# baggepinnen/LPVSpectral.jl

Measured on AMD Instinct MI355X. Metric: signals/sec, ls_sparse_spectral_lpv group lasso N=2^20 Nf=512 Nv=8 (2000 ADMM iters; iters/sec in admm_iters_per_sec), higher is better.
Workload: dtype f64

## Files before the change

### lpvspectral.jl_amd/csrc/api.hip

```cpp
#include <cmath>
#include <cstdarg>
#include <cstdio>
#include <cstdlib>
#include <cstring>
#include <ctime>
#include <map>
#include <mutex>
#include <array>
#include <thread>
#include <string>
#include <vector>

#include "lpvs_internal.h"

namespace lpvs {

static thread_local char g_err[512] = "";

void set_error(const char *fmt, ...) {
    va_list ap;
    va_start(ap, fmt);
    vsnprintf(g_err, sizeof(g_err), fmt, ap);
    va_end(ap);
}
// ... 872 lines not shown
    sl.s0 = sl.nf8;
    bool merged = false;
    if (Nf > 1 && D != 0.0L) {
        const long double j0r = 2.0L * a0 / D;
        const long long j0 = llroundl(j0r);
        const long double delta = 2.0L * a0 - (long double)j0 * D;
        if (j0 >= 0 && j0 < Nf && std::fabs((double)delta) * xam <= 1e-7) {
            merged = true; sl.merged = true;
            sl.s0 = j0; sl.delta = (double)delta;
            sl.nsl = round_up(j0 + 2 * Nf - 1, 8);
            sl.s8 = sl.nsl;
        }
    }
    sl.om_hi.resize((size_t)sl.nsl); sl.om_lo.resize((size_t)sl.nsl);
    if (merged) {
        for (int64_t j = 0; j < sl.nsl; ++j) split((long double)j * D, sl.om_hi[j], sl.om_lo[j]);
    } else {
        for (int64_t m = 0; m < sl.nf8; ++m) split((long double)m * D, sl.om_hi[m], sl.om_lo[m]);
        for (int64_t q = 0; q < sl.s8; ++q) split(2.0L * a0 + (long double)q * D, sl.om_hi[sl.nf8 + q], sl.om_lo[sl.nf8 + q]);
    }
    for (int64_t f = 0; f < sl.nf8; ++f) split(a0 + (long double)f * D, sl.omr_hi[f], sl.omr_lo[f]);
    for (int b = 0; b < 8; ++b) split((long double)b * D, sl.step.hi[b], sl.step.lo[b]);
    return sl;
}
struct ApSlotsDev {
    DevBuf hi, lo, rhi, rlo, eps;
    int32_t upload(const ApSlots &sl, hipStream_t s) {
        LPVS_TRY(hi.alloc(sizeof(double) * (size_t)sl.nsl)); LPVS_TRY(lo.alloc(sizeof(double) * (size_t)sl.nsl));
        LPVS_TRY(rhi.alloc(sizeof(double) * (size_t)sl.nf8)); LPVS_TRY(rlo.alloc(sizeof(double) * (size_t)sl.nf8));
        LPVS_TRY(eps.alloc(sizeof(double) * sl.eps.size()));
        LPVS_TRY(copy_to_device(hi.p, sl.om_hi.data(), sizeof(double) * (size_t)sl.nsl, s));
        LPVS_TRY(copy_to_device(lo.p, sl.om_lo.data(), sizeof(double) * (size_t)sl.nsl, s));
        LPVS_TRY(copy_to_device(rhi.p, sl.omr_hi.data(), sizeof(double) * (size_t)sl.nf8, s));
        LPVS_TRY(copy_to_device(rlo.p, sl.omr_lo.data(), sizeof(double) * (size_t)sl.nf8, s));
        LPVS_TRY(copy_to_device(eps.p, sl.eps.data(), sizeof(double) * sl.eps.size(), s));
        return LPVS_OK;
    }
};

static int32_t create_lpv_impl(const double *y, int64_t ns, const double *X, const double *V, int64_t N, const double *w, int64_t Nf,
                               int64_t Nv, int32_t normalize, int32_t coulomb, int32_t device, lpvs_problem **out,
                               const double *ranges = nullptr) {
    if (N <= 0 || Nf <= 0 || Nv <= 0 || ns <= 0) { set_error("N, Nf, Nv and the number of signals must be positive"); return LPVS_EARGUMENT; }
    lpvs_problem *h = nullptr;
    LPVS_TRY(problem_begin(device, out, &h));
    struct Guard { lpvs_problem *h; ~Guard() { delete h; } } guard{h};
    hipStream_t s = h->stream;
    const int64_t nb = coulomb ? 2 * Nv : Nv;
    h->kind = 1; h->N = N; h->Nf = Nf; h->nb = nb; h->n = 2 * Nf * nb; h->np = round_up(h->n, 128); h->ns = ns;
    DevArg dy, dX, dV, dw;
    LPVS_TRY(dy.set(y, N * ns, s)); LPVS_TRY(dX.set(X, N, s)); LPVS_TRY(dV.set(V, N, s)); LPVS_TRY(dw.set(w, Nf, s));
    LPVS_TRY(h->G.alloc(sizeof(double) * (size_t)h->np * (size_t)h->np));
    LPVS_TRY(h->b.alloc(sizeof(double) * (size_t)h->np * (size_t)ns));
    LPVS_HIP(hipMemsetAsync(h->G.p, 0, h->G.bytes, s));
    LPVS_HIP(hipMemsetAsync(h->b.p, 0, h->b.bytes, s));
    LPVS_TRY(alloc_state(h));

    const int form_opt = option_in_effect(LPVS_OPT_GRAM_FORM, h->opt[LPVS_OPT_GRAM_FORM]);
    const std::string form = form_opt == LPVS_GRAM_AP ? "ap" : form_opt == LPVS_GRAM_KRS ? "krs" : form_opt == LPVS_GRAM_KR ? "kr" : "auto";
    bool use_ap = false;
    ApSlots sl;
    double xam = 0;
    if (form == "auto" || form == "ap") {
        std::vector<double> hw;
        LPVS_TRY(fetch_host(hw, w, Nf));
        double xlo, xhi;
        if (ranges) xam = ranges[3];
        else LPVS_TRY(device_minmax(dX.p, N, &xlo, &xhi, &xam, s));
        sl = make_ap_slots(hw, xam);
        use_ap = sl.ok;
        if (form == "ap" && !use_ap) { set_error("LPVS_GRAM_FORM=ap but w is not an arithmetic progression (max|eps|*max|x| = %.3g)", sl.emax * xam); return LPVS_EARGUMENT; }
    }
    if (use_ap) {
        const int64_t nf8 = sl.nf8, nsl = sl.nsl, P = nb * (nb + 1) / 2;
        const ApStep &step = sl.step;
        double lo, hi, am, gamma; std::vector<double> vc;
        DevBuf K, KK, dvc, part, tab, tabb, nwork, epsr;
        ApSlotsDev sd;
        DrainOnExit drain(s);
        LPVS_HIP(hipEventRecord(h->ev[0].a, s));
        if (ranges) { lo = ranges[0]; hi = ranges[1]; am = ranges[2]; }
        else LPVS_TRY(device_minmax(dV.p, N, &lo, &hi, &am, s));
        basis_centers(lo, hi, am, Nv, coulomb, vc, &gamma);
        const int64_t ldk = nb + 1;
        LPVS_TRY(dvc.alloc(sizeof(double) * vc.size()));
        LPVS_TRY(copy_to_device(dvc.p, vc.data(), sizeof(double) * vc.size(), s));
        LPVS_TRY(K.alloc(sizeof(double) * (size_t)N * (size_t)ldk));
        LPVS_TRY(KK.alloc(sizeof(double) * (size_t)N * (size_t)P));
        LPVS_TRY(launch_basis_table(dV.p, N, dvc.as<double>(), nb, gamma, normalize, coulomb, K.as<double>(), ldk, s));
        LPVS_TRY(launch_pair_table(K.as<double>(), ldk, nb, N, KK.as<double>(), s));
        LPVS_TRY(sd.upload(sl, s));
        LPVS_HIP(hipEventRecord(h->ev[0].b, s));
        LPVS_TRY(part.alloc(std::max(nudft_partial_bytes(N, nsl, P), nudft_partial_bytes(N, nf8, nb))));
        LPVS_TRY(tab.alloc(sizeof(double) * (size_t)nsl * (size_t)P * 4));
        LPVS_TRY(tabb.alloc(sizeof(double) * (size_t)nf8 * (size_t)nb * 4));
        LPVS_HIP(hipEventRecord(h->ev[1].a, s));
        const bool nufft_on = option_in_effect(LPVS_OPT_SLOT_SUMS, h->opt[LPVS_OPT_SLOT_SUMS]) != LPVS_SLOTS_DIRECT;
        bool nufft = nufft_on && sl.merged && nufft_applicable(N, nsl, P);
        const int nfg = nufft_grid_size(nsl);
        const double xam_ = xam;
        if (nufft) {
            LPVS_TRY(nwork.alloc(nufft_work_bytes(N, nsl, P)));
            const int32_t rc = launch_nufft_tab(dX.p, nullptr, N, xam_, KK.as<double>(), P, (int)P, step.hi[1], step.lo[1], 0, (int)nsl, nfg, false, nwork.p,
                                                tab.as<double>(), s);
            if (rc == kNufftNonFinite) nufft = false;
            else if (rc != LPVS_OK) return rc;
        }
        if (nufft) {
            h->gram_form = 5;
        } else {
            h->gram_form = 4;
            LPVS_TRY(launch_nudft(dX.p, nullptr, N, KK.as<double>(), P, (int)P, sd.hi.as<double>(), sd.lo.as<double>(), (int)nsl, step, part.as<double>(), tab.as<double>(), s));
        }
        LPVS_TRY(launch_ap_assemble(tab.as<double>(), sd.eps.as<double>(), Nf, sl.s0, sl.delta, nb, h->n, h->G.as<double>(), h->np, s));
        LPVS_HIP(hipEventRecord(h->ev[1].b, s));
        LPVS_HIP(hipEventRecord(h->ev[2].a, s));
        const bool nufft_rhs = nufft && sl.s0 % 2 == 0 && (int)(sl.s0 / 2 + nf8) <= (int)nsl;
        if (nufft_rhs) {
            std::vector<double> er(sl.eps.size());
            for (size_t f = 0; f < er.size(); ++f) er[f] = sl.eps[f] + 0.5 * sl.delta;
            LPVS_TRY(epsr.alloc(sizeof(double) * er.size()));
            LPVS_TRY(copy_to_device(epsr.p, er.data(), sizeof(double) * er.size(), s));
            LPVS_HIP(hipStreamSynchronize(s));
        }
// ... 1527 lines not shown
```

### lpvspectral.jl_amd/csrc/nudft.hip

```cpp
#include "lpvs_internal.h"

#include <cstdlib>

namespace lpvs {

namespace {

constexpr int RB = 16;

template <int QPT, int S>
__global__ void __launch_bounds__(256)
nudft_accumulate_kernel(const double *__restrict__ x, const double *__restrict__ y, int64_t N, const double *__restrict__ Wt,
                        int64_t ldw, int nq, const double *__restrict__ om_hi, const double *__restrict__ om_lo, int nslots,
                        const ApStep step, double *__restrict__ out, const int64_t *__restrict__ seg, int64_t rows_per_chunk) {
    constexpr int SLOTS = 64 * S, NA = 8 * S;
    constexpr int WSTR = (QPT + 1) & ~1;
    constexpr int NEF = NA + 8;
    __shared__ __attribute__((aligned(16))) double wrow[2][RB][4 * WSTR];
    __shared__ __attribute__((aligned(16))) double ef[2][RB][NEF][2];
    __shared__ double xs[2][RB], ys[2][RB];
    const int t = threadIdx.x;
    const int sl = t & 63;
    const int g = __builtin_amdgcn_readfirstlane(t >> 6);
    const int slot0 = blockIdx.x * SLOTS;
// ... 181 lines not shown
    }
}

__global__ void __launch_bounds__(256)
nudft_reduce_kernel(const double *__restrict__ part_all, int nchunks, int64_t count, double *__restrict__ out_all) {
    const int64_t i = (int64_t)blockIdx.x * 256 + threadIdx.x;
    if (i >= count) return;
    const double *part = part_all + (int64_t)blockIdx.y * nchunks * count;
    double s = 0;
    for (int c = 0; c < nchunks; ++c) s += part[(int64_t)c * count + i];
    out_all[(int64_t)blockIdx.y * count + i] = s;
}

__global__ void __launch_bounds__(256)
ap_assemble_fourier_kernel(const double *__restrict__ tab_all, const double *__restrict__ eps, int Nf, int s0, double delta, int zf, double scale,
                           int64_t n, double *__restrict__ G_all, int64_t ldg, int64_t tab_stride, int64_t g_stride) {
    const int64_t ga = blockIdx.y;
    const int64_t gb = (int64_t)blockIdx.x * 256 + threadIdx.x;
    if (gb > ga || ga >= n) return;
    const double *tab = tab_all + (int64_t)blockIdx.z * tab_stride;
    double *G = G_all + (int64_t)blockIdx.z * g_stride;
    const int ca = ga >= Nf, cb = gb >= Nf;
    const int ka = ca ? (int)ga - Nf + zf : (int)ga, kb = cb ? (int)gb - Nf + zf : (int)gb;
    const int hi = ka >= kb ? ka : kb, lo = ka >= kb ? kb : ka;
    const double dm = eps[hi] - eps[lo], dp = (eps[ka] + eps[kb]) + delta;
    const double *tm = tab + (int64_t)(hi - lo) * 4;
    const double *tp = tab + (int64_t)(s0 + ka + kb) * 4;
    const double cm = fma(-dm, tm[3], tm[0]);
    double sm = fma(dm, tm[2], tm[1]);
    if (ka < kb) sm = -sm;
    const double cp = fma(-dp, tp[3], tp[0]), sp = fma(dp, tp[2], tp[1]);
    double v;
    if (!ca && !cb) v = 0.5 * (cm + cp);
    else if (ca && cb) v = 0.5 * (cm - cp);
    else if (!ca && cb) v = -0.5 * (sp - sm);
    else v = -0.5 * (sp + sm);
    v *= scale;
    G[ga * ldg + gb] = v;
    G[gb * ldg + ga] = v;
}

__global__ void __launch_bounds__(256)
ap_rhs_fourier_kernel(const double *__restrict__ tab_all, const double *__restrict__ eps, int Nf, int zf, double dd,
                      double *__restrict__ b_all, int64_t tab_stride, int64_t b_stride) {
    const int k = blockIdx.x * 256 + threadIdx.x;
    if (k >= Nf) return;
    const double *t = tab_all + (int64_t)blockIdx.y * tab_stride + (int64_t)k * 4;
    double *b = b_all + (int64_t)blockIdx.y * b_stride;
    const double e = eps[k];
    b[k] = dd * fma(-e, t[3], t[0]);
    if (k >= zf) b[Nf + k - zf] = -dd * fma(e, t[2], t[1]);
}

__global__ void __launch_bounds__(256)
ap_assemble_kernel(const double *__restrict__ tab, const double *__restrict__ eps, int Nf, int s0, double delta, int nb, int P, int64_t n,
                   double *__restrict__ G, int64_t ldg) {
    const int64_t ga = blockIdx.y;
    const int64_t gb = (int64_t)blockIdx.x * 256 + threadIdx.x;
    if (gb > ga || ga >= n) return;
    const int g2 = 2 * nb;
    const int fa = (int)(ga / g2), ra = (int)(ga - (int64_t)fa * g2), ca = ra >= nb, ja0 = ra - ca * nb;
    const int fb = (int)(gb / g2), rbm = (int)(gb - (int64_t)fb * g2), cb = rbm >= nb, jb0 = rbm - cb * nb;
    int ja = ja0, jb = jb0;
    if (ja > jb) { const int t = ja; ja = jb; jb = t; }
    const int q = ja * nb - ja * (ja - 1) / 2 + (jb - ja);
    const int m = fa - fb, s = fa + fb;
    const double dm = eps[fa] - eps[fb], dp = (eps[fa] + eps[fb]) + delta;
    const double *tm = tab + ((int64_t)m * P + q) * 4;
    const double *tp = tab + ((int64_t)(s0 + s) * P + q) * 4;
    const double cm = fma(-dm, tm[3], tm[0]), sm = fma(dm, tm[2], tm[1]);
    const double cp = fma(-dp, tp[3], tp[0]), sp = fma(dp, tp[2], tp[1]);
    double v;
    if (!ca && !cb) v = 0.5 * (cm + cp);
    else if (ca && cb) v = 0.5 * (cm - cp);
    else if (!ca && cb) v = -0.5 * (sp - sm);
    else v = -0.5 * (sp + sm);
    G[ga * ldg + gb] = v;
    G[gb * ldg + ga] = v;
}

__global__ void __launch_bounds__(256)
ap_rhs_kernel(const double *__restrict__ tab, const double *__restrict__ eps, int Nf, int nb, double *__restrict__ b) {
    const int i = blockIdx.x * 256 + threadIdx.x;
    if (i >= Nf * nb) return;
    const int f = i / nb, j = i - f * nb;
    const double *t = tab + ((int64_t)f * nb + j) * 4;
    const double e = eps[f];
    b[(int64_t)f * 2 * nb + j] = fma(-e, t[3], t[0]);
    b[(int64_t)f * 2 * nb + nb + j] = -fma(e, t[2], t[1]);
}

template <int QPT, int S>
void launch_accumulate(unsigned nchunks, hipStream_t s, const double *x, const double *y, int64_t N, const double *Wt, int64_t ldw, int nq,
                       const double *om_hi, const double *om_lo, int nslots, const ApStep &step, double *partial, const int64_t *seg,
                       int64_t rpc) {
    dim3 grid((unsigned)ceil_div(nslots, 64 * S), nchunks, (unsigned)ceil_div(nq, 4 * QPT));
    hipLaunchKernelGGL((nudft_accumulate_kernel<QPT, S>), grid, dim3(256), 0, s, x, y, N, Wt, ldw, nq, om_hi, om_lo, nslots, step, partial, seg, rpc);
}

}

int64_t nudft_rows_per_chunk(int64_t N, int64_t nslots) {
    const int64_t groups = ceil_div(nslots, 128);
    int64_t rpc = 8192;
    while (rpc > 64 && groups * ceil_div(N, rpc) < 2048) rpc >>= 1;
    return rpc;
}
size_t nudft_chunks(int64_t N, int64_t nslots) { return (size_t)ceil_div(N, nudft_rows_per_chunk(N, nslots)); }
size_t nudft_partial_bytes(int64_t N, int64_t nslots, int64_t nq) {
    return sizeof(double) * nudft_chunks(N, nslots) * (size_t)nslots * (size_t)nq * 4;
}

static int32_t nudft_impl(const double *x, const double *y, int64_t N, const double *Wt, int64_t ldw, int nq, const double *om_hi,
                          const double *om_lo, int nslots, const ApStep &step, double *partial, double *tab, const int64_t *seg,
                          unsigned nseg, unsigned nbatch, hipStream_t s) {
    if (nslots % 8 != 0) { set_error("nudft: slot count %d is not a multiple of 8", nslots); return LPVS_ESTATE; }
    const unsigned nchunks = seg ? nseg : (unsigned)nudft_chunks(N, nslots);
    const int64_t rpc = seg ? 0 : nudft_rows_per_chunk(N, nslots);
    if (nq == 1) {
        dim3 grid((unsigned)ceil_div(nslots, 128), nchunks, 1);
        hipLaunchKernelGGL(nudft_single_kernel<2>, grid, dim3(256), 0, s, x, y, N, Wt, ldw, om_hi, om_lo, nslots, step, partial, seg, rpc);
    } else if (nq <= 8) launch_accumulate<2, 2>(nchunks, s, x, y, N, Wt, ldw, nq, om_hi, om_lo, nslots, step, partial, seg, rpc);
    else if (nq <= 16) launch_accumulate<4, 2>(nchunks, s, x, y, N, Wt, ldw, nq, om_hi, om_lo, nslots, step, partial, seg, rpc);
    else launch_accumulate<9, 2>(nchunks, s, x, y, N, Wt, ldw, nq, om_hi, om_lo, nslots, step, partial, seg, rpc);
    LPVS_HIP(hipGetLastError());
    const int64_t count = (int64_t)nslots * nq * 4;
    hipLaunchKernelGGL(nudft_reduce_kernel, dim3((unsigned)ceil_div(count, 256), nbatch), dim3(256), 0, s, partial, (int)(nchunks / nbatch), count, tab);
    LPVS_HIP(hipGetLastError());
    return LPVS_OK;
}

int32_t launch_nudft(const double *x, const double *y, int64_t N, const double *Wt, int64_t ldw, int nq, const double *om_hi,
                     const double *om_lo, int nslots, const ApStep &step, double *partial, double *tab, hipStream_t s) {
    return nudft_impl(x, y, N, Wt, ldw, nq, om_hi, om_lo, nslots, step, partial, tab, nullptr, 0, 1, s);
}

int32_t launch_nudft_windows(const double *x, const double *y, const double *Wt, const double *om_hi, const double *om_lo, int nslots,
                             const ApStep &step, const int64_t *seg_dev, int nwin, int segs_per_window, double *partial, double *tab,
                             hipStream_t s) {
    return nudft_impl(x, y, 0, Wt, 1, 1, om_hi, om_lo, nslots, step, partial, tab, seg_dev, (unsigned)(nwin * segs_per_window), (unsigned)nwin, s);
}

int32_t launch_ap_assemble_fourier(const double *tab, const double *eps, int64_t Nf, int64_t s0, double delta, int zf, int64_t n, double *G,
                                   int64_t ldg, int nbatch, int64_t tab_stride, int64_t g_stride, hipStream_t s) {
    dim3 grid((unsigned)ceil_div(n, 256), (unsigned)n, (unsigned)nbatch);
    hipLaunchKernelGGL(ap_assemble_fourier_kernel, grid, dim3(256), 0, s, tab, eps, (int)Nf, (int)s0, delta, zf, 1.0 / (double)(2 * Nf), n, G, ldg,
                       tab_stride, g_stride);
    LPVS_HIP(hipGetLastError());
    return LPVS_OK;
}

int32_t launch_ap_rhs_fourier(const double *tab, const double *eps, int64_t Nf, int zf, double *b, int nbatch, int64_t tab_stride,
                              int64_t b_stride, hipStream_t s) {
    hipLaunchKernelGGL(ap_rhs_fourier_kernel, dim3((unsigned)ceil_div(Nf, 256), (unsigned)nbatch), dim3(256), 0, s, tab, eps, (int)Nf, zf,
                       1.0 / sqrt((double)(2 * Nf)), b, tab_stride, b_stride);
    LPVS_HIP(hipGetLastError());
    return LPVS_OK;
}

int32_t launch_ap_assemble(const double *tab, const double *eps, int64_t Nf, int64_t s0, double delta, int64_t nb, int64_t n, double *G,
                           int64_t ldg, hipStream_t s) {
    const int P = (int)(nb * (nb + 1) / 2);
    dim3 grid((unsigned)ceil_div(n, 256), (unsigned)n);
    hipLaunchKernelGGL(ap_assemble_kernel, grid, dim3(256), 0, s, tab, eps, (int)Nf, (int)s0, delta, (int)nb, P, n, G, ldg);
    LPVS_HIP(hipGetLastError());
    return LPVS_OK;
}

int32_t launch_ap_rhs(const double *tab, const double *eps, int64_t Nf, int64_t nb, double *b, hipStream_t s) {
    hipLaunchKernelGGL(ap_rhs_kernel, dim3((unsigned)ceil_div(Nf * nb, 256)), dim3(256), 0, s, tab, eps, (int)Nf, (int)nb, b);
    LPVS_HIP(hipGetLastError());
    return LPVS_OK;
}

}
```

### lpvspectral.jl_amd/csrc/nufft.hip

```cpp
#include "lpvs_internal.h"

#include <cmath>
#include <map>
#include <mutex>
#include <vector>

namespace lpvs {
namespace {

constexpr int NU_W = 16;
constexpr double NU_BETA = 2.30 * NU_W;
static int nu_gpw(int nf) { return nf <= 4096 ? 4 : 2; }
constexpr double NU_MAGIC = 6755399441055744.0;
constexpr int NU_CHUNK = 32768;

__global__ void __launch_bounds__(256)
nufft_coord_kernel(const double *__restrict__ x, int64_t N, double D_hi, double D_lo, int nf, int *__restrict__ cell0, double *__restrict__ taps) {
    const int64_t i = (int64_t)blockIdx.x * 256 + threadIdx.x;
    if (i >= N) return;
    constexpr double I2PI_HI = 0.15915494309189535, I2PI_LO = -9.8393384885635288e-18;
    const double xv = x[i];
    const double th = D_hi * xv, tl = fma(D_hi, xv, -th) + D_lo * xv;
    const double uh = th * I2PI_HI, ul = fma(th, I2PI_HI, -uh) + (th * I2PI_LO + tl * I2PI_HI);
    double r = (uh - rint(uh)) + ul;
    r -= floor(r);
    double p = r * (double)nf;
    if (p >= (double)nf) p -= (double)nf;
    const int g0 = (int)ceil(p - 0.5 * NU_W);
    cell0[i] = (g0 + nf) & (nf - 1);
#pragma unroll
    for (int k = 0; k < NU_W; ++k) {
        const double z = ((double)(g0 + k) - p) * (2.0 / NU_W);
        const double s = 1.0 - z * z;
        taps[i * NU_W + k] = s > 0.0 ? exp(NU_BETA * (sqrt(s) - 1.0)) : exp(-NU_BETA);
    }
}

__global__ void __launch_bounds__(256)
nufft_colmax_kernel(const double *__restrict__ Wt, const double *__restrict__ y, int64_t ldw, int nq, int64_t N, unsigned long long *__restrict__ out) {
    __shared__ unsigned long long m[256];
    for (int q = threadIdx.x; q < 256; q += 256) m[q] = 0;
    __syncthreads();
    const int64_t total = N * ldw;
    for (int64_t e = (int64_t)blockIdx.x * 256 + threadIdx.x; e < total; e += (int64_t)gridDim.x * 256) {
        const int q = (int)(e % ldw);
        if (q < nq) {
            const double v = fabs(y ? Wt[e] * y[e / ldw] : Wt[e]);
            if (v > 0.0 || v != v) atomicMax(&m[q & 255], v != v ? 0x7ff0000000000000ull : (unsigned long long)__double_as_longlong(v));
        }
    }
    __syncthreads();
    for (int q = threadIdx.x; q < nq && q < 256; q += 256) if (m[q]) atomicMax(out + q, m[q]);
}

template <int GPW>
__global__ void __launch_bounds__(256)
nufft_spread_kernel(const double *__restrict__ x, const double *__restrict__ y, const double *__restrict__ Wt, int64_t ldw, int nq, int64_t N, int nf,
                    const int *__restrict__ cell0, const double *__restrict__ taps, const double *__restrict__ invq,
                    long long *__restrict__ partial, int ngroups, int nchunks) {
    extern __shared__ __attribute__((aligned(16))) long long G[];
    const int xcd = blockIdx.x & 7, jj = blockIdx.x >> 3;
    const int gg = jj % ngroups, ch = xcd + 8 * (jj / ngroups);
    if (ch >= nchunks) return;
    for (int e = threadIdx.x; e < GPW * nf; e += 256) G[e] = 0;
    __syncthreads();
    constexpr int NC = GPW / 2;
    const int q0 = gg * NC;
    double iq[GPW];
#pragma unroll
    for (int c = 0; c < NC; ++c) { iq[2 * c] = q0 + c < nq ? invq[2 * (q0 + c)] : 0.0; iq[2 * c + 1] = q0 + c < nq ? invq[2 * (q0 + c) + 1] : 0.0; }
    const int64_t n0 = (int64_t)ch * NU_CHUNK, n1 = n0 + NU_CHUNK < N ? n0 + NU_CHUNK : N;
    const long long magic_bits = __double_as_longlong(NU_MAGIC);
    for (int64_t n = n0 + threadIdx.x; n < n1; n += 256) {
        const int c0 = cell0[n];
        const double xv = x[n], yv = y ? y[n] : 1.0;
        double cw[GPW];
#pragma unroll
        for (int c = 0; c < NC; ++c) {
            const double wv = q0 + c < nq ? Wt[n * ldw + q0 + c] * yv : 0.0;
            cw[2 * c] = wv * iq[2 * c];
            cw[2 * c + 1] = (xv * wv) * iq[2 * c + 1];
        }
        const double2 *tp = reinterpret_cast<const double2 *>(taps + n * NU_W);
#pragma unroll
        for (int k2 = 0; k2 < NU_W / 2; ++k2) {
            const double2 t = tp[k2];
#pragma unroll
            for (int h = 0; h < 2; ++h) {
                const double tv = h ? t.y : t.x;
                const int cell = (c0 + 2 * k2 + h) & (nf - 1);
#pragma unroll
                for (int gi = 0; gi < GPW; ++gi) {
                    const long long a = __double_as_longlong(fma(cw[gi], tv, NU_MAGIC)) - magic_bits;
                    atomicAdd(reinterpret_cast<unsigned long long *>(&G[gi * nf + cell]), (unsigned long long)a);
                }
            }
        }
    }
    __syncthreads();
    long long *out = partial + ((int64_t)ch * ngroups + gg) * GPW * nf;
    for (int e = threadIdx.x; e < GPW * nf; e += 256) out[e] = G[e];
}

__global__ void __launch_bounds__(256)
nufft_reduce_kernel(const long long *__restrict__ partial, int ngroups, int nchunks, int nf, int gpw, double *__restrict__ grid) {
    const int gamma = blockIdx.y, q = gamma >> 1, twin = gamma & 1;
    const int gg = q / (gpw / 2), gi = (q % (gpw / 2)) * 2 + twin;
    const int g = blockIdx.x * 256 + threadIdx.x;
    if (g >= nf) return;
    long long s = 0;
    for (int ch = 0; ch < nchunks; ++ch) s += partial[(((int64_t)ch * ngroups + gg) * gpw + gi) * nf + g];
    grid[(int64_t)gamma * nf + g] = (double)s;
}

template <bool HALF>
__global__ void __launch_bounds__(256)
nufft_modes_kernel(const double *__restrict__ grid, int nf, int nq, int mode0, int nslots,
                   const double *__restrict__ scale , double *__restrict__ tab,
                   int64_t scale_stride , int64_t grid_bstride, int64_t tab_bstride ) {
    grid += (int64_t)blockIdx.z * grid_bstride;
    tab += (int64_t)blockIdx.z * tab_bstride;
    extern __shared__ __attribute__((aligned(16))) double lds[];
    double *Gd = lds;
    double2 *tw = reinterpret_cast<double2 *>(lds + nf);
    const int gamma = blockIdx.x, q = gamma >> 1, twin = gamma & 1;
    const int ntw = HALF ? nf >> 1 : nf;
    for (int g = threadIdx.x; g < nf; g += 256) {
        Gd[g] = grid[(int64_t)gamma * nf + g];
        if (g < ntw) {
            double sn, cs;
            sincospi(2.0 * (double)g / (double)nf, &sn, &cs);
            tw[g] = make_double2(cs, sn);
        }
    }
    __syncthreads();
    const int j = blockIdx.y * 256 + threadIdx.x;
    if (j >= nslots) return;
    double ac0 = 0, as0 = 0, ac1 = 0, as1 = 0;
    int idx = 0;
    const int mask = nf - 1, mj = (mode0 + j) & mask;
    const int hmask = mask >> 1, hbit = nf >> 1;
    for (int g = 0; g < nf; g += 2) {
        const double2 t0 = tw[HALF ? idx & hmask : idx];
        const bool n0 = HALF && (idx & hbit);
        idx = (idx + mj) & mask;
        const double2 t1 = tw[HALF ? idx & hmask : idx];
        const bool n1 = HALF && (idx & hbit);
        idx = (idx + mj) & mask;
        double v0 = Gd[g], v1 = Gd[g + 1];
        if (HALF) { v0 = n0 ? -v0 : v0; v1 = n1 ? -v1 : v1; }
        ac0 = fma(v0, t0.x, ac0); as0 = fma(v0, t0.y, as0);
        ac1 = fma(v1, t1.x, ac1); as1 = fma(v1, t1.y, as1);
    }
    const double sc = scale[(int64_t)gamma * scale_stride + j];
// ... 75 lines not shown
    }
}

}

static std::vector<long double> nufft_phihat(int nf, int nmodes) {
    static const std::vector<std::pair<long double, long double>> gl = [] {
        const int n = 96;
        std::vector<std::pair<long double, long double>> r((size_t)n);
        const long double pi = 3.141592653589793238462643383279502884L;
        for (int i = 0; i < n; ++i) {
            long double z = cosl(pi * (i + 0.75L) / (n + 0.5L)), pp = 0;
            for (int it = 0; it < 100; ++it) {
                long double p1 = 1, p2 = 0;
                for (int k = 1; k <= n; ++k) { const long double p3 = p2; p2 = p1; p1 = ((2 * k - 1) * z * p2 - (k - 1) * p3) / k; }
                pp = n * (z * p1 - p2) / (z * z - 1);
                const long double dz = p1 / pp;
                z -= dz;
                if (fabsl(dz) < 1e-19L) break;
            }
            r[(size_t)i] = {z, 2 / ((1 - z * z) * pp * pp)};
        }
        return r;
    }();
    static std::mutex phat_mu;
    static std::map<std::pair<int, int>, std::vector<long double>> phat_cache;
    std::lock_guard<std::mutex> lk(phat_mu);
    auto it = phat_cache.find({nf, nmodes});
    if (it == phat_cache.end()) {
        std::vector<long double> v((size_t)nmodes);
        const long double pi = 3.141592653589793238462643383279502884L, half = 0.5L * NU_W;
        for (int j = 0; j < nmodes; ++j) {
            long double acc = 0;
            for (const auto &nw : gl) {
                const long double z = nw.first, t = z * half;
                acc += nw.second * half * expl((long double)NU_BETA * (sqrtl(1 - z * z) - 1)) * cosl(2 * pi * (long double)j * t / (long double)nf);
            }
            v[(size_t)j] = acc;
        }
        it = phat_cache.emplace(std::make_pair(nf, nmodes), std::move(v)).first;
    }
    return it->second;
}

int nufft_grid_size(int64_t nslots) {
    int nf = 256;
    while ((double)nf < 3.9 * (double)nslots) nf *= 2;
    return nf;
}
bool nufft_applicable(int64_t N, int64_t nslots, int64_t nq) {
    const int nf = nufft_grid_size(nslots);
    return nf <= 8192 && N >= 4096 && nq >= 1 && nq <= 256;
}
size_t nufft_work_bytes(int64_t N, int64_t nslots, int64_t nq) {
    const int nf = nufft_grid_size(nslots), gpw = nu_gpw(nf);
    const int64_t ngroups = (nq + gpw / 2 - 1) / (gpw / 2), nchunks = (N + NU_CHUNK - 1) / NU_CHUNK;
    size_t b = 0;
    b += sizeof(double) * (size_t)N * NU_W;
    b += ((sizeof(int) * (size_t)N + 255) / 256) * 256;
    b += sizeof(long long) * (size_t)nchunks * (size_t)ngroups * (size_t)gpw * (size_t)nf;
    b += sizeof(double) * (size_t)(2 * nq) * (size_t)(nslots + 1);
    b += sizeof(double) * (size_t)(2 * nq) * (size_t)nf;
    b += sizeof(unsigned long long) * (size_t)nq + 256;
    return b;
}

int32_t launch_nufft_tab(const double *x, const double *y, int64_t N, double xam, const double *Wt, int64_t ldw, int nq, double D_hi, double D_lo,
                         int mode0, int nslots, int nf, bool reuse_coords, void *work, double *tab, hipStream_t s) {
    const int gpw = nu_gpw(nf);
    const int ngroups = (nq + gpw / 2 - 1) / (gpw / 2), nchunks = (int)((N + NU_CHUNK - 1) / NU_CHUNK);
    unsigned char *wp = static_cast<unsigned char *>(work);
    double *taps = reinterpret_cast<double *>(wp); wp += sizeof(double) * (size_t)N * NU_W;
    int *cell0 = reinterpret_cast<int *>(wp); wp += ((sizeof(int) * (size_t)N + 255) / 256) * 256;
    long long *partial = reinterpret_cast<long long *>(wp); wp += sizeof(long long) * (size_t)nchunks * (size_t)ngroups * (size_t)gpw * (size_t)nf;
    double *scale = reinterpret_cast<double *>(wp); wp += sizeof(double) * (size_t)(2 * nq) * (size_t)nslots;
    double *invq = reinterpret_cast<double *>(wp); wp += sizeof(double) * (size_t)(2 * nq);
    double *grid = reinterpret_cast<double *>(wp); wp += sizeof(double) * (size_t)(2 * nq) * (size_t)nf;
    unsigned long long *colmax = reinterpret_cast<unsigned long long *>(wp);

    LPVS_HIP(hipMemsetAsync(colmax, 0, sizeof(unsigned long long) * (size_t)nq, s));
    if (!reuse_coords) hipLaunchKernelGGL(nufft_coord_kernel, dim3((unsigned)ceil_div(N, 256)), dim3(256), 0, s, x, N, D_hi, D_lo, nf, cell0, taps);
    if (nq > 256) { set_error("nufft: more than 256 weight vectors"); return LPVS_EUNSUPPORTED; }
    hipLaunchKernelGGL(nufft_colmax_kernel, dim3(1024), dim3(256), 0, s, Wt, y, ldw, nq, N, colmax);
    LPVS_HIP(hipGetLastError());
    std::vector<unsigned long long> hm((size_t)nq);
    LPVS_HIP(hipMemcpyAsync(hm.data(), colmax, sizeof(unsigned long long) * (size_t)nq, hipMemcpyDeviceToHost, s));
    LPVS_HIP(hipStreamSynchronize(s));
    for (int q = 0; q < nq; ++q)
        if (!std::isfinite(__builtin_bit_cast(double, hm[(size_t)q])) || !std::isfinite(xam)) return kNufftNonFinite;
    std::vector<double> hscale((size_t)(2 * nq) * (size_t)nslots), hinvq((size_t)(2 * nq));
    const std::vector<long double> phat = nufft_phihat(nf, mode0 + nslots);
    for (int q = 0; q < nq; ++q) {
        const double cmax = __builtin_bit_cast(double, hm[(size_t)q]);
        for (int twin = 0; twin < 2; ++twin) {
            const double bound = (twin ? xam : 1.0) * cmax * (double)N;
            int e = 0;
            (void)std::frexp(bound > 0 ? bound : 1.0, &e);
            const double quantum = std::ldexp(1.0, e - 62);
            hinvq[(size_t)(2 * q + twin)] = bound > 0 ? 1.0 / quantum : 0.0;
            for (int j = 0; j < nslots; ++j) hscale[(size_t)(2 * q + twin) * (size_t)nslots + (size_t)j] = (double)((long double)quantum / phat[(size_t)(mode0 + j)]);
        }
    }
    LPVS_TRY(copy_to_device(scale, hscale.data(), sizeof(double) * hscale.size(), s));
    LPVS_TRY(copy_to_device(invq, hinvq.data(), sizeof(double) * hinvq.size(), s));
    const size_t lds_spread = sizeof(long long) * (size_t)gpw * (size_t)nf;
    if (gpw == 4) {
        LPVS_HIP(hipFuncSetAttribute(reinterpret_cast<const void *>(&nufft_spread_kernel<4>), hipFuncAttributeMaxDynamicSharedMemorySize, (int)lds_spread));
        hipLaunchKernelGGL(nufft_spread_kernel<4>, dim3((unsigned)(8 * ngroups * ceil_div(nchunks, 8))), dim3(256), lds_spread, s, x, y, Wt, ldw, nq, N, nf, cell0,
                           taps, invq, partial, ngroups, nchunks);
    } else {
        LPVS_HIP(hipFuncSetAttribute(reinterpret_cast<const void *>(&nufft_spread_kernel<2>), hipFuncAttributeMaxDynamicSharedMemorySize, (int)lds_spread));
        hipLaunchKernelGGL(nufft_spread_kernel<2>, dim3((unsigned)(8 * ngroups * ceil_div(nchunks, 8))), dim3(256), lds_spread, s, x, y, Wt, ldw, nq, N, nf, cell0,
                           taps, invq, partial, ngroups, nchunks);
    }
    hipLaunchKernelGGL(nufft_reduce_kernel, dim3((unsigned)ceil_div(nf, 256), (unsigned)(2 * nq)), dim3(256), 0, s, partial, ngroups, nchunks, nf, gpw, grid);
    if (nf <= 4096) {
        const size_t lds_modes = sizeof(double) * 3 * (size_t)nf;
        LPVS_HIP(hipFuncSetAttribute(reinterpret_cast<const void *>(&nufft_modes_kernel<false>), hipFuncAttributeMaxDynamicSharedMemorySize, (int)lds_modes));
        hipLaunchKernelGGL(nufft_modes_kernel<false>, dim3((unsigned)(2 * nq), (unsigned)ceil_div(nslots, 256)), dim3(256), lds_modes, s, grid, nf, nq, mode0,
                           nslots, scale, tab, (int64_t)nslots, (int64_t)0, (int64_t)0);
    } else {
        const size_t lds_modes = sizeof(double) * 2 * (size_t)nf;
        LPVS_HIP(hipFuncSetAttribute(reinterpret_cast<const void *>(&nufft_modes_kernel<true>), hipFuncAttributeMaxDynamicSharedMemorySize, (int)lds_modes));
        hipLaunchKernelGGL(nufft_modes_kernel<true>, dim3((unsigned)(2 * nq), (unsigned)ceil_div(nslots, 256)), dim3(256), lds_modes, s, grid, nf, nq, mode0,
                           nslots, scale, tab, (int64_t)nslots, (int64_t)0, (int64_t)0);
    }
    LPVS_HIP(hipGetLastError());
    return LPVS_OK;
}


bool nufft_windows_applicable(int64_t n, int64_t nslots) {
    return n >= 2048 && nslots >= 64 && nufft_grid_size(nslots) <= 4096;
}
std::vector<double> nufft_window_scale(int nf, int mode0, int nslots) {
    const std::vector<long double> phat = nufft_phihat(nf, mode0 + nslots);
    std::vector<double> r((size_t)nslots);
    for (int j = 0; j < nslots; ++j) r[(size_t)j] = (double)(1.0L / phat[(size_t)(mode0 + j)]);
    return r;
}
int32_t launch_nufft_window_spread(const double *x, const double *W, const double *yA, const double *yB, bool hasB, const int64_t *offs_dev, int nwin,
                                   int64_t n, double D_hi, double D_lo, int nf, double *gridA, double *gridB, int64_t grid_bstride, hipStream_t s) {
    const size_t lds = sizeof(long long) * 4 * (size_t)nf;
    LPVS_HIP(hipFuncSetAttribute(reinterpret_cast<const void *>(&nufft_window_kernel), hipFuncAttributeMaxDynamicSharedMemorySize, (int)lds));
    hipLaunchKernelGGL(nufft_window_kernel, dim3((unsigned)nwin), dim3(256), lds, s, x, W, yA, yB, hasB ? 1 : 0, offs_dev, n, D_hi, D_lo, nf, gridA, gridB,
                       grid_bstride);
    LPVS_HIP(hipGetLastError());
    return LPVS_OK;
}
int32_t launch_nufft_window_modes(const double *grids, int64_t grid_bstride, int nwin, int nf, int mode0, int nslots, const double *scale_dev, double *tab,
                                  int64_t tab_bstride, hipStream_t s) {
    const size_t lds_modes = sizeof(double) * 3 * (size_t)nf;
    LPVS_HIP(hipFuncSetAttribute(reinterpret_cast<const void *>(&nufft_modes_kernel<false>), hipFuncAttributeMaxDynamicSharedMemorySize, (int)lds_modes));
    hipLaunchKernelGGL(nufft_modes_kernel<false>, dim3(2, (unsigned)ceil_div(nslots, 256), (unsigned)nwin), dim3(256), lds_modes, s, grids, nf, 1, mode0, nslots,
                       scale_dev, tab, (int64_t)0, grid_bstride, tab_bstride);
    LPVS_HIP(hipGetLastError());
    return LPVS_OK;
}

}
```

Measured before the change: 15.20.

## Bin NUFFT samples by cell and gather, tile Gram assembly, trim memsets

The NUFFT spreading step now sorts samples into per-cell bins with a counting sort and runs a gather kernel by default. Each thread accumulates its own cell in fixed-point registers, replacing the LDS scatter, which remains available through an environment switch. The AP Gram assembly now uses 32x32 tiles with an LDS transpose so the mirrored writes are coalesced. The full Gram memset becomes a memset of only the padding region, and building the host-side scale table is moved after the kernel launches so it can overlap GPU work. All of this touches only setup, not the ADMM iterations, so it adds binning cost and more complexity in exchange.

```diff
diff --git a/lpvspectral.jl_amd/csrc/api.hip b/lpvspectral.jl_amd/csrc/api.hip
--- a/lpvspectral.jl_amd/csrc/api.hip
+++ b/lpvspectral.jl_amd/csrc/api.hip
@@ -948,7 +948,6 @@
     LPVS_TRY(dy.set(y, N * ns, s)); LPVS_TRY(dX.set(X, N, s)); LPVS_TRY(dV.set(V, N, s)); LPVS_TRY(dw.set(w, Nf, s));
     LPVS_TRY(h->G.alloc(sizeof(double) * (size_t)h->np * (size_t)h->np));
     LPVS_TRY(h->b.alloc(sizeof(double) * (size_t)h->np * (size_t)ns));
-    LPVS_HIP(hipMemsetAsync(h->G.p, 0, h->G.bytes, s));
     LPVS_HIP(hipMemsetAsync(h->b.p, 0, h->b.bytes, s));
     LPVS_TRY(alloc_state(h));
 
@@ -966,6 +965,15 @@
         sl = make_ap_slots(hw, xam);
         use_ap = sl.ok;
         if (form == "ap" && !use_ap) { set_error("LPVS_GRAM_FORM=ap but w is not an arithmetic progression (max|eps|*max|x| = %.3g)", sl.emax * xam); return LPVS_EARGUMENT; }
+    }
+    if (use_ap) {
+        const int64_t n = h->n, np = h->np;
+        if (np > n) {
+            LPVS_HIP(hipMemsetAsync(h->G.as<double>() + n * np, 0, sizeof(double) * (size_t)(np - n) * (size_t)np, s));
+            LPVS_HIP(hipMemset2DAsync(h->G.as<double>() + n, sizeof(double) * (size_t)np, 0, sizeof(double) * (size_t)(np - n), (size_t)n, s));
+        }
+    } else {
+        LPVS_HIP(hipMemsetAsync(h->G.p, 0, h->G.bytes, s));
     }
     if (use_ap) {
         const int64_t nf8 = sl.nf8, nsl = sl.nsl, P = nb * (nb + 1) / 2;
diff --git a/lpvspectral.jl_amd/csrc/nudft.hip b/lpvspectral.jl_amd/csrc/nudft.hip
--- a/lpvspectral.jl_amd/csrc/nudft.hip
+++ b/lpvspectral.jl_amd/csrc/nudft.hip
@@ -257,12 +257,8 @@
     if (k >= zf) b[Nf + k - zf] = -dd * fma(e, t[2], t[1]);
 }
 
-__global__ void __launch_bounds__(256)
-ap_assemble_kernel(const double *__restrict__ tab, const double *__restrict__ eps, int Nf, int s0, double delta, int nb, int P, int64_t n,
-                   double *__restrict__ G, int64_t ldg) {
-    const int64_t ga = blockIdx.y;
-    const int64_t gb = (int64_t)blockIdx.x * 256 + threadIdx.x;
-    if (gb > ga || ga >= n) return;
+__device__ __forceinline__ double ap_gram_value(const double *__restrict__ tab, const double *__restrict__ eps, int s0, double delta, int nb, int P,
+                                                int64_t ga, int64_t gb) {
     const int g2 = 2 * nb;
     const int fa = (int)(ga / g2), ra = (int)(ga - (int64_t)fa * g2), ca = ra >= nb, ja0 = ra - ca * nb;
     const int fb = (int)(gb / g2), rbm = (int)(gb - (int64_t)fb * g2), cb = rbm >= nb, jb0 = rbm - cb * nb;
@@ -280,8 +276,34 @@
     else if (ca && cb) v = 0.5 * (cm - cp);
     else if (!ca && cb) v = -0.5 * (sp - sm);
     else v = -0.5 * (sp + sm);
-    G[ga * ldg + gb] = v;
-    G[gb * ldg + ga] = v;
+    return v;
+}
+constexpr int AP_TILE = 32;
+__global__ void __launch_bounds__(256)
+ap_assemble_kernel(const double *__restrict__ tab, const double *__restrict__ eps, int Nf, int s0, double delta, int nb, int P, int64_t n,
+                   double *__restrict__ G, int64_t ldg) {
+    (void)Nf;
+    if (blockIdx.x > blockIdx.y) return;
+    __shared__ double tile[AP_TILE][AP_TILE + 1];
+    const int tx = threadIdx.x & (AP_TILE - 1), ty = threadIdx.x / AP_TILE;
+    const int64_t row0 = (int64_t)blockIdx.y * AP_TILE, col0 = (int64_t)blockIdx.x * AP_TILE;
+#pragma unroll
+    for (int u = 0; u < AP_TILE / 8; ++u) {
+        const int r = ty + 8 * u;
+        const int64_t ga = row0 + r, gb = col0 + tx;
+        if (ga < n && gb <= ga) {
+            const double v = ap_gram_value(tab, eps, s0, delta, nb, P, ga, gb);
+            tile[r][tx] = v;
+            G[ga * ldg + gb] = v;
+        }
+    }
+    __syncthreads();
+#pragma unroll
+    for (int u = 0; u < AP_TILE / 8; ++u) {
+        const int r = ty + 8 * u;
+        const int64_t R = col0 + r, C = row0 + tx;
+        if (C < n && R < C) G[R * ldg + C] = tile[tx][r];
+    }
 }
 
 __global__ void __launch_bounds__(256)
@@ -366,7 +388,7 @@
 int32_t launch_ap_assemble(const double *tab, const double *eps, int64_t Nf, int64_t s0, double delta, int64_t nb, int64_t n, double *G,
                            int64_t ldg, hipStream_t s) {
     const int P = (int)(nb * (nb + 1) / 2);
-    dim3 grid((unsigned)ceil_div(n, 256), (unsigned)n);
+    dim3 grid((unsigned)ceil_div(n, AP_TILE), (unsigned)ceil_div(n, AP_TILE));
     hipLaunchKernelGGL(ap_assemble_kernel, grid, dim3(256), 0, s, tab, eps, (int)Nf, (int)s0, delta, (int)nb, P, n, G, ldg);
     LPVS_HIP(hipGetLastError());
     return LPVS_OK;
diff --git a/lpvspectral.jl_amd/csrc/nufft.hip b/lpvspectral.jl_amd/csrc/nufft.hip
--- a/lpvspectral.jl_amd/csrc/nufft.hip
+++ b/lpvspectral.jl_amd/csrc/nufft.hip
@@ -1,6 +1,8 @@
 #include "lpvs_internal.h"
+#include "nufft_bins.h"
 
 #include <cmath>
+#include <cstring>
 #include <map>
 #include <mutex>
 #include <vector>
@@ -8,11 +10,11 @@
 namespace lpvs {
 namespace {
 
-constexpr int NU_W = 16;
+constexpr int NU_W = kNuWidth;
 constexpr double NU_BETA = 2.30 * NU_W;
-static int nu_gpw(int nf) { return nf <= 4096 ? 4 : 2; }
+static int nu_gpw(int nf) { return nu_scatter_gpw(nf); }
 constexpr double NU_MAGIC = 6755399441055744.0;
-constexpr int NU_CHUNK = 32768;
+constexpr int NU_CHUNK = kNuChunk;
 
 __global__ void __launch_bounds__(256)
 nufft_coord_kernel(const double *__restrict__ x, int64_t N, double D_hi, double D_lo, int nf, int *__restrict__ cell0, double *__restrict__ taps) {
@@ -100,6 +102,109 @@
     __syncthreads();
     long long *out = partial + ((int64_t)ch * ngroups + gg) * GPW * nf;
     for (int e = threadIdx.x; e < GPW * nf; e += 256) out[e] = G[e];
+}
+
+
+__global__ void __launch_bounds__(256)
+nufft_bin_kernel(const int *__restrict__ cell0, int64_t N, int nf, int *__restrict__ bin_start, int *__restrict__ perm) {
+    extern __shared__ __attribute__((aligned(16))) int cnt[];
+    __shared__ int part[256];
+    const int64_t base = (int64_t)blockIdx.x * kNuBinChunk;
+    const int count = (int)(N - base < kNuBinChunk ? N - base : kNuBinChunk);
+    for (int e = threadIdx.x; e < nf; e += 256) cnt[e] = 0;
+    __syncthreads();
+    for (int i = threadIdx.x; i < count; i += 256) atomicAdd(&cnt[cell0[base + i]], 1);
+    __syncthreads();
+    const int per = nf / 256, e0 = threadIdx.x * per;
+    int sum = 0;
+    for (int e = 0; e < per; ++e) sum += cnt[e0 + e];
+    part[threadIdx.x] = sum;
+    __syncthreads();
+    for (int d = 1; d < 256; d <<= 1) {
+        const int v = threadIdx.x >= d ? part[threadIdx.x - d] : 0;
+        __syncthreads();
+        part[threadIdx.x] += v;
+        __syncthreads();
+    }
+    int run = part[threadIdx.x] - sum;
+    int *bs = bin_start + (int64_t)blockIdx.x * (nf + 1);
+    for (int e = 0; e < per; ++e) { const int c = cnt[e0 + e]; cnt[e0 + e] = run; bs[e0 + e] = run; run += c; }
+    if (threadIdx.x == 255) bs[nf] = run;
+    __syncthreads();
+    for (int i = threadIdx.x; i < count; i += 256) perm[base + atomicAdd(&cnt[cell0[base + i]], 1)] = i;
+}
+
+__global__ void __launch_bounds__(256)
+nufft_gather_kernel(const double *__restrict__ x, const double *__restrict__ y, const double *__restrict__ Wt, int64_t ldw, int nq, int64_t N, int nf,
+                    const int *__restrict__ cell0, const double *__restrict__ taps, const int *__restrict__ perm, const int *__restrict__ bin_start,
+                    const double *__restrict__ invq, long long *__restrict__ partial, NuGatherPlan plan) {
+    constexpr int G = kNuGatherGrids, NC = G / 2, T = kNuStage;
+    __shared__ double s_cw[G][T];
+    __shared__ int2 s_cs[T];
+    const NuGatherBlock blk = nu_gather_block(plan, blockIdx.x);
+    if (!blk.valid) return;
+    const int c = blk.cellblock * kNuCellBlock + threadIdx.x;
+    const int q0 = blk.group * NC;
+    double iq[G];
+#pragma unroll
+    for (int j = 0; j < NC; ++j) { iq[2 * j] = q0 + j < nq ? invq[2 * (q0 + j)] : 0.0; iq[2 * j + 1] = q0 + j < nq ? invq[2 * (q0 + j) + 1] : 0.0; }
+    unsigned long long acc[G];
+#pragma unroll
+    for (int gi = 0; gi < G; ++gi) acc[gi] = 0;
+    unsigned long long naddends = 0;
+    constexpr int RUNS = kNuChunk / kNuBinChunk;
+    for (int sub = 0; sub < RUNS; ++sub) {
+        const int64_t run = (int64_t)blk.chunk * RUNS + sub, base = run * kNuBinChunk;
+        if (base >= N) break;
+        const int *bs = bin_start + run * (nf + 1);
+        const NuRanges mine = nu_cell_ranges(bs, nf, c, 1), block = nu_cell_ranges(bs, nf, blk.cellblock * kNuCellBlock, kNuCellBlock);
+        for (int seg = 0; seg < 2; ++seg)
+            for (int t0 = block.r[seg].lo; t0 < block.r[seg].hi; t0 += T) {
+                const int t1 = t0 + T < block.r[seg].hi ? t0 + T : block.r[seg].hi;
+                __syncthreads();
+                for (int p = t0 + threadIdx.x; p < t1; p += 256) {
+                    const int ls = perm[base + p];
+                    const int64_t n = base + ls;
+                    const double xv = x[n], yv = y ? y[n] : 1.0;
+                    s_cs[p - t0] = make_int2(cell0[n], ls);
+#pragma unroll
+                    for (int j = 0; j < NC; ++j) {
+                        const double wv = q0 + j < nq ? Wt[n * ldw + q0 + j] * yv : 0.0;
+                        s_cw[2 * j][p - t0] = wv * iq[2 * j];
+                        s_cw[2 * j + 1][p - t0] = (xv * wv) * iq[2 * j + 1];
+                    }
+                }
+                __syncthreads();
+#pragma unroll
+                for (int r = 0; r < 2; ++r) {
+                    const int lo = mine.r[r].lo > t0 ? mine.r[r].lo : t0, hi = mine.r[r].hi < t1 ? mine.r[r].hi : t1;
+                    for (int p = lo; p < hi; p += 4) {
+                        int idx[4];
+                        double tv[4];
+#pragma unroll
+                        for (int u = 0; u < 4; ++u) {
+                            idx[u] = (p + u < hi ? p + u : hi - 1) - t0;
+                            const int2 cs = s_cs[idx[u]];
+                            tv[u] = taps[(base + cs.y) * NU_W + nu_tap_index(c, cs.x, nf)];
+                        }
+#pragma unroll
+                        for (int u = 0; u < 4; ++u) {
+                            const double t = p + u < hi ? tv[u] : 0.0;
+#pragma unroll
+                            for (int gi = 0; gi < G; ++gi)
+                                acc[gi] += (unsigned long long)__double_as_longlong(fma(s_cw[gi][idx[u]], t, NU_MAGIC));
+                        }
+                        naddends += 4;
+                    }
+                }
+            }
+    }
+    const unsigned long long off = naddends * (unsigned long long)__double_as_longlong(NU_MAGIC);
+#pragma unroll
+    for (int gi = 0; gi < G; ++gi) {
+        const int gamma = blk.group * G + gi;
+        if (gamma < 2 * nq) partial[((int64_t)blk.chunk * plan.padded_grids + gamma) * nf + c] = (long long)(acc[gi] - off);
+    }
 }
 
 __global__ void __launch_bounds__(256)
@@ -281,34 +386,31 @@
     const int nf = nufft_grid_size(nslots);
     return nf <= 8192 && N >= 4096 && nq >= 1 && nq <= 256;
 }
-size_t nufft_work_bytes(int64_t N, int64_t nslots, int64_t nq) {
-    const int nf = nufft_grid_size(nslots), gpw = nu_gpw(nf);
-    const int64_t ngroups = (nq + gpw / 2 - 1) / (gpw / 2), nchunks = (N + NU_CHUNK - 1) / NU_CHUNK;
-    size_t b = 0;
-    b += sizeof(double) * (size_t)N * NU_W;
-    b += ((sizeof(int) * (size_t)N + 255) / 256) * 256;
-    b += sizeof(long long) * (size_t)nchunks * (size_t)ngroups * (size_t)gpw * (size_t)nf;
-    b += sizeof(double) * (size_t)(2 * nq) * (size_t)(nslots + 1);
-    b += sizeof(double) * (size_t)(2 * nq) * (size_t)nf;
-    b += sizeof(unsigned long long) * (size_t)nq + 256;
-    return b;
-}
+size_t nufft_work_bytes(int64_t N, int64_t nslots, int64_t nq) { return nu_work_layout(N, nufft_grid_size(nslots), nslots, nq).total; }
 
 int32_t launch_nufft_tab(const double *x, const double *y, int64_t N, double xam, const double *Wt, int64_t ldw, int nq, double D_hi, double D_lo,
                          int mode0, int nslots, int nf, bool reuse_coords, void *work, double *tab, hipStream_t s) {
     const int gpw = nu_gpw(nf);
     const int ngroups = (nq + gpw / 2 - 1) / (gpw / 2), nchunks = (int)((N + NU_CHUNK - 1) / NU_CHUNK);
+    const bool scatter = [] { const char *e = experiment_env("LPVS_NUFFT_SPREAD"); return e && strcmp(e, "scatter") == 0; }();
+    const NuWork lay = nu_work_layout(N, nf, nslots, nq);
     unsigned char *wp = static_cast<unsigned char *>(work);
-    double *taps = reinterpret_cast<double *>(wp); wp += sizeof(double) * (size_t)N * NU_W;
-    int *cell0 = reinterpret_cast<int *>(wp); wp += ((sizeof(int) * (size_t)N + 255) / 256) * 256;
-    long long *partial = reinterpret_cast<long long *>(wp); wp += sizeof(long long) * (size_t)nchunks * (size_t)ngroups * (size_t)gpw * (size_t)nf;
-    double *scale = reinterpret_cast<double *>(wp); wp += sizeof(double) * (size_t)(2 * nq) * (size_t)nslots;
-    double *invq = reinterpret_cast<double *>(wp); wp += sizeof(double) * (size_t)(2 * nq);
-    double *grid = reinterpret_cast<double *>(wp); wp += sizeof(double) * (size_t)(2 * nq) * (size_t)nf;
-    unsigned long long *colmax = reinterpret_cast<unsigned long long *>(wp);
+    double *taps = reinterpret_cast<double *>(wp + lay.taps);
+    int *cell0 = reinterpret_cast<int *>(wp + lay.cell0);
+    int *perm = reinterpret_cast<int *>(wp + lay.perm);
+    int *bin_start = reinterpret_cast<int *>(wp + lay.bin_start);
+    long long *partial = reinterpret_cast<long long *>(wp + lay.partial);
+    double *scale = reinterpret_cast<double *>(wp + lay.scale);
+    double *invq = reinterpret_cast<double *>(wp + lay.invq);
+    double *grid = reinterpret_cast<double *>(wp + lay.grid);
+    unsigned long long *colmax = reinterpret_cast<unsigned long long *>(wp + lay.colmax);
 
     LPVS_HIP(hipMemsetAsync(colmax, 0, sizeof(unsigned long long) * (size_t)nq, s));
-    if (!reuse_coords) hipLaunchKernelGGL(nufft_coord_kernel, dim3((unsigned)ceil_div(N, 256)), dim3(256), 0, s, x, N, D_hi, D_lo, nf, cell0, taps);
+    if (!reuse_coords) {
+        hipLaunchKernelGGL(nufft_coord_kernel, dim3((unsigned)ceil_div(N, 256)), dim3(256), 0, s, x, N, D_hi, D_lo, nf, cell0, taps);
+        if (!scatter)
+            hipLaunchKernelGGL(nufft_bin_kernel, dim3((unsigned)ceil_div(N, kNuBinChunk)), dim3(256), sizeof(int) * (size_t)nf, s, cell0, N, nf, bin_start, perm);
+    }
     if (nq > 256) { set_error("nufft: more than 256 weight vectors"); return LPVS_EUNSUPPORTED; }
     hipLaunchKernelGGL(nufft_colmax_kernel, dim3(1024), dim3(256), 0, s, Wt, y, ldw, nq, N, colmax);
     LPVS_HIP(hipGetLastError());
@@ -317,8 +419,7 @@
     LPVS_HIP(hipStreamSynchronize(s));
     for (int q = 0; q < nq; ++q)
         if (!std::isfinite(__builtin_bit_cast(double, hm[(size_t)q])) || !std::isfinite(xam)) return kNufftNonFinite;
-    std::vector<double> hscale((size_t)(2 * nq) * (size_t)nslots), hinvq((size_t)(2 * nq));
-    const std::vector<long double> phat = nufft_phihat(nf, mode0 + nslots);
+    std::vector<double> hquantum((size_t)(2 * nq)), hinvq((size_t)(2 * nq));
     for (int q = 0; q < nq; ++q) {
         const double cmax = __builtin_bit_cast(double, hm[(size_t)q]);
         for (int twin = 0; twin < 2; ++twin) {
@@ -326,14 +427,17 @@
             int e = 0;
             (void)std::frexp(bound > 0 ? bound : 1.0, &e);
             const double quantum = std::ldexp(1.0, e - 62);
+            hquantum[(size_t)(2 * q + twin)] = quantum;
             hinvq[(size_t)(2 * q + twin)] = bound > 0 ? 1.0 / quantum : 0.0;
-            for (int j = 0; j < nslots; ++j) hscale[(size_t)(2 * q + twin) * (size_t)nslots + (size_t)j] = (double)((long double)quantum / phat[(size_t)(mode0 + j)]);
-        }
-    }
-    LPVS_TRY(copy_to_device(scale, hscale.data(), sizeof(double) * hscale.size(), s));
+        }
+    }
     LPVS_TRY(copy_to_device(invq, hinvq.data(), sizeof(double) * hinvq.size(), s));
     const size_t lds_spread = sizeof(long long) * (size_t)gpw * (size_t)nf;
-    if (gpw == 4) {
+    if (!scatter) {
+        const NuGatherPlan plan = nu_gather_plan(N, nf, nq);
+        hipLaunchKernelGGL(nufft_gather_kernel, dim3((unsigned)plan.nblocks), dim3(256), 0, s, x, y, Wt, ldw, nq, N, nf, cell0, taps, perm, bin_start, invq,
+                           partial, plan);
+    } else if (gpw == 4) {
         LPVS_HIP(hipFuncSetAttribute(reinterpret_cast<const void *>(&nufft_spread_kernel<4>), hipFuncAttributeMaxDynamicSharedMemorySize, (int)lds_spread));
         hipLaunchKernelGGL(nufft_spread_kernel<4>, dim3((unsigned)(8 * ngroups * ceil_div(nchunks, 8))), dim3(256), lds_spread, s, x, y, Wt, ldw, nq, N, nf, cell0,
                            taps, invq, partial, ngroups, nchunks);
@@ -343,6 +447,14 @@
                            taps, invq, partial, ngroups, nchunks);
     }
     hipLaunchKernelGGL(nufft_reduce_kernel, dim3((unsigned)ceil_div(nf, 256), (unsigned)(2 * nq)), dim3(256), 0, s, partial, ngroups, nchunks, nf, gpw, grid);
+    LPVS_HIP(hipGetLastError());
+    {
+        std::vector<double> hscale((size_t)(2 * nq) * (size_t)nslots);
+        const std::vector<long double> phat = nufft_phihat(nf, mode0 + nslots);
+        for (int g = 0; g < 2 * nq; ++g)
+            for (int j = 0; j < nslots; ++j) hscale[(size_t)g * (size_t)nslots + (size_t)j] = (double)((long double)hquantum[(size_t)g] / phat[(size_t)(mode0 + j)]);
+        LPVS_TRY(copy_to_device(scale, hscale.data(), sizeof(double) * hscale.size(), s));
+    }
     if (nf <= 4096) {
         const size_t lds_modes = sizeof(double) * 3 * (size_t)nf;
         LPVS_HIP(hipFuncSetAttribute(reinterpret_cast<const void *>(&nufft_modes_kernel<false>), hipFuncAttributeMaxDynamicSharedMemorySize, (int)lds_modes));
diff --git a/lpvspectral.jl_amd/csrc/nufft_bins.h b/lpvspectral.jl_amd/csrc/nufft_bins.h
--- /dev/null
+++ b/lpvspectral.jl_amd/csrc/nufft_bins.h
@@ -0,0 +1,87 @@
+#pragma once
+
+#include <cstddef>
+#include <cstdint>
+
+#if defined(__HIPCC__)
+#define LPVS_NU_HD __host__ __device__
+#else
+#define LPVS_NU_HD
+#endif
+
+namespace lpvs {
+
+constexpr int kNuWidth = 16;
+constexpr int kNuChunk = 32768;
+constexpr int kNuBinChunk = 4096;
+constexpr int kNuCellBlock = 256;
+constexpr int kNuGatherGrids = 8;
+constexpr int kNuStage = 512;
+
+LPVS_NU_HD inline int nu_scatter_gpw(int nf) { return nf <= 4096 ? 4 : 2; }
+
+struct NuRange { int lo, hi; };
+struct NuRanges { NuRange r[2]; };
+template <class BinStart>
+LPVS_NU_HD inline NuRanges nu_cell_ranges(const BinStart &bin_start, int nf, int first, int count) {
+    NuRanges o;
+    const int b0 = first - (kNuWidth - 1);
+    if (count + (kNuWidth - 1) >= nf) { o.r[0] = {bin_start[0], bin_start[nf]}; o.r[1] = {0, 0}; }
+    else if (b0 >= 0) { o.r[0] = {bin_start[b0], bin_start[first + count]}; o.r[1] = {0, 0}; }
+    else { o.r[0] = {bin_start[b0 + nf], bin_start[nf]}; o.r[1] = {bin_start[0], bin_start[first + count]}; }
+    return o;
+}
+LPVS_NU_HD inline int nu_tap_index(int c, int cell0, int nf) { return (c - cell0) & (nf - 1); }
+
+struct NuGatherPlan {
+    int nchunks, nbinchunks, ncellblocks, ngroups;
+    int padded_grids;
+    int64_t nblocks;
+};
+LPVS_NU_HD inline NuGatherPlan nu_gather_plan(int64_t N, int nf, int nq) {
+    NuGatherPlan p;
+    const int gpw = nu_scatter_gpw(nf);
+    p.nchunks = (int)((N + kNuChunk - 1) / kNuChunk);
+    p.nbinchunks = (int)((N + kNuBinChunk - 1) / kNuBinChunk);
+    p.ncellblocks = nf / kNuCellBlock;
+    p.ngroups = (2 * nq + kNuGatherGrids - 1) / kNuGatherGrids;
+    p.padded_grids = (2 * nq + gpw - 1) / gpw * gpw;
+    const int64_t units = (int64_t)p.nchunks * p.ncellblocks;
+    p.nblocks = 8 * (int64_t)p.ngroups * ((units + 7) / 8);
+    return p;
+}
+struct NuGatherBlock { int chunk, cellblock, group; bool valid; };
+LPVS_NU_HD inline NuGatherBlock nu_gather_block(const NuGatherPlan &p, int64_t block) {
+    const int xcd = (int)(block & 7);
+    const int64_t jj = block >> 3;
+    const int64_t unit = xcd + 8 * (jj / p.ngroups);
+    NuGatherBlock b;
+    b.group = (int)(jj % p.ngroups);
+    b.valid = unit < (int64_t)p.nchunks * p.ncellblocks;
+    b.chunk = (int)(unit / p.ncellblocks);
+    b.cellblock = (int)(unit % p.ncellblocks);
+    return b;
+}
+
+struct NuWork {
+    size_t taps, cell0, perm, bin_start, partial, scale, invq, grid, colmax, total;
+};
+inline size_t nu_align256(size_t b) { return (b + 255) / 256 * 256; }
+inline NuWork nu_work_layout(int64_t N, int nf, int64_t nslots, int64_t nq) {
+    const NuGatherPlan p = nu_gather_plan(N, nf, (int)nq);
+    NuWork w;
+    size_t b = 0;
+    w.taps = b;      b += nu_align256(sizeof(double) * (size_t)N * kNuWidth);
+    w.cell0 = b;     b += nu_align256(sizeof(int) * (size_t)N);
+    w.perm = b;      b += nu_align256(sizeof(int) * (size_t)N);
+    w.bin_start = b; b += nu_align256(sizeof(int) * (size_t)p.nbinchunks * (size_t)(nf + 1));
+    w.partial = b;   b += nu_align256(sizeof(long long) * (size_t)p.nchunks * (size_t)p.padded_grids * (size_t)nf);
+    w.scale = b;     b += nu_align256(sizeof(double) * (size_t)(2 * nq) * (size_t)nslots);
+    w.invq = b;      b += nu_align256(sizeof(double) * (size_t)(2 * nq));
+    w.grid = b;      b += nu_align256(sizeof(double) * (size_t)(2 * nq) * (size_t)nf);
+    w.colmax = b;    b += nu_align256(sizeof(unsigned long long) * (size_t)nq);
+    w.total = b;
+    return w;
+}
+
+}
```

Result: faster. 15.48, median of 6 (+1.9%).
